# theogf/AugmentedGaussianProcesses.jl

Measured on AMD Instinct MI355X. Metric: cavi_iters_per_sec, higher is better.
Workload: dtype f64

## Files before the change

augmentedgaussianprocesses.jl_amd/csrc/agp_capi.hip:

```cpp
#include "../../include/agp_hip.h"

#include <hip/hip_runtime.h>

#include <algorithm>
#include <cmath>
#include <cstdio>
#include <cstring>
#include <string>
#include <vector>

#include "agp_cavi.h"
#include "agp_comm.h"
#include "agp_hyper.h"
#include "agp_kmeans.h"
#include "agp_linalg.h"

using namespace agp;

struct agp_ctx {
  int device = 0;
  hipStream_t stream = nullptr;
  std::string err;
  int32_t* dag_flags = nullptr;
  int64_t dag_cap = 0;
// ... 17 lines not shown
  int32_t* safe_retries = nullptr;
  int n_cu = 0;
  bool dag_off = false;
  int64_t dag_retries_seen = 0;
  int64_t dag_cooldown = 0, dag_backoff = 512;
  hipStream_t side = nullptr;
  hipEvent_t ev_fork = nullptr, ev_join = nullptr;
  void* chol_li = nullptr;
  size_t chol_li_bytes = 0;
  hipStream_t chain_stream = nullptr;
  int32_t* chain_go = nullptr;
  int32_t* chain_ctr = nullptr;
  int32_t chain_exits = 0;
  int chain_state = 0;
  int32_t chain_seq = 0;
};

#define HIPCHK(ctx, expr)                                                                       \
  do {                                                                                          \
    hipError_t _e = (expr);                                                                     \
    if (_e != hipSuccess) {                                                                     \
      (ctx)->err = std::string(#expr) + " : " + hipGetErrorString(_e);                          \
      return AGP_ERR_HIP;                                                                       \
    }                                                                                           \
  } while (0)

#define LAUNCHCHK(ctx)                                                                          \
  do {                                                                                          \
    hipError_t _e = hipGetLastError();                                                          \
    if (_e != hipSuccess) {                                                                     \
      (ctx)->err = std::string("kernel launch : ") + hipGetErrorString(_e) + " @" + std::to_string(__LINE__); \
// ... 158 lines not shown
  LAUNCHCHK(c);
  return AGP_OK;
}
template <typename T>
__global__ __launch_bounds__(CHOL_THREADS) void k_safe_rowstats(CholBatch<T> bt, SafeSrc<T> src, int64_t ld, int64_t ldx, int64_t lde,
                                                                int64_t ne, int64_t nt, int32_t* __restrict__ info, int64_t nvalid,
                                                                unsigned* __restrict__ bar, int32_t* __restrict__ retries,
                                                                int64_t B, int nslices, RowstatsBatch<T> rb, int64_t ldp,
                                                                int64_t ldw, int64_t cols, T jitter, T rho, LikParams<T> lp,
                                                                const T* __restrict__ y, const int64_t* __restrict__ idx,
                                                                T* __restrict__ Kt, T* __restrict__ muf, T* __restrict__ varf,
                                                                T* __restrict__ cb, T* __restrict__ theta, T* __restrict__ r,
                                                                T* __restrict__ w, int* __restrict__ flags,
                                                                const T* __restrict__ lam, T* __restrict__ gamma,
                                                                int rows_done = 0, const int32_t* __restrict__ pf_word = nullptr,
                                                                int32_t pf_want = 0) {
  __shared__ __attribute__((aligned(16))) T sm[3 * TILE * LDP];
  __shared__ __attribute__((aligned(16))) T sc[SC_ELEMS];
  __shared__ T piv[TILE];
  const bool ran = chol_safe_body<T>(bt, src, 1, ld, ldx, lde, ne, nt, info, nvalid, bar, retries, sm, sc, piv);
  if (ran || !rows_done) {
    const int64_t wpb = CHOL_THREADS / 64, nwave = (int64_t)gridDim.x * wpb;
    for (int64_t i = (int64_t)blockIdx.x * wpb + (threadIdx.x >> 6); i < B; i += nwave)
      rowstats_row<T>(i, threadIdx.x & 63, 0, B, nslices, rb, ldp, ldw, cols, jitter, rho, lp, y, idx, Kt, muf, varf, cb, theta, r,
                      w, (int64_t)0, flags, lam, gamma);
  }
  if (pf_word && blockIdx.x == 0 && threadIdx.x == 0) {
    long spins = 0;
    while ((int32_t)(__hip_atomic_load(pf_word, __ATOMIC_RELAXED, __HIP_MEMORY_SCOPE_SYSTEM) - pf_want) < 0) {
      __builtin_amdgcn_s_sleep(8);
      if (++spins > (1L << 27)) {
        atomicExch(info, -2);
        break;
      }
    }
  }
}

template <typename T>
__global__ __launch_bounds__(CHOL_THREADS) void k_safe_symv_trmv(CholBatch<T> bt, SafeSrc<T> src, int64_t ld, int64_t ldx, int64_t lde,
// ... 195 lines not shown
struct ProHost {
  const T* kap = nullptr;
  int64_t ldk = 0, Kdim = 0;
  const T *w = nullptr, *r = nullptr;
  T* eta2 = nullptr;
  const T* Kinv = nullptr;
  int64_t ldm = 0;
  T* eta1 = nullptr;
  const T* kinv_mu0 = nullptr;
  T lr = T(0);
  const T *packed = nullptr, *tred = nullptr;
  const int32_t* arrive = nullptr;
  int32_t arrive_want = 0;
  unsigned char grp[32] = {};
  T* Cout = nullptr;
};
static void pro_ks_table(int64_t nt, int64_t nq, bool f64, unsigned char* ks, unsigned char* kf) {
  const double tc = f64 ? 2.7 : 1.6, tau = f64 ? 17.8 : 14.0;
  for (int64_t c = 0; c < nt && c < 32; ++c) {
    int want;
    if (c == 0) want = 8;
    else if (c == 1) want = f64 ? 4 : 8;
    else want = (int)std::ceil((double)nq * (tc + 0.3) / (tau * (double)c - 12.0));
    want = std::max(1, std::min<int>(want, (int)std::min<int64_t>(8, nq)));
    ks[c] = kf[c] = (unsigned char)want;
  }
}
static bool dag_test_abort() {
  static const bool on = []() {
    const char* e = getenv("AGP_DAG_TEST_ABORT");
    return e && e[0] == '1';
  }();
  return on;
}

template <typename T>
static agp_status potrf_fused(agp_ctx* c, T* A, int64_t ld, int64_t n, T* X, int64_t ldx, T* Dg, T* E, int64_t lde,
                              int64_t ne, int do_x, int32_t* info_dev, int64_t nvalid, const T* erow = nullptr,
// ... 6 lines not shown
  const int64_t nt = n / TILE;
  const bool use_dag = chol_use_dag(c, nt, ne);
  bool split_used = false;
  if (pro && !(use_dag && X && !want_l && nt <= 32)) {
    c->err = "potrf_fused: a pending natural-gradient step can only ride on the CAVI step's task-graph launch";
    return AGP_ERR_INVALID;
  }
  if (use_dag && X) {
    const int64_t nx = (do_x && nt > 1) ? nt : 0;
    ProArgs<T> pa{};
    int64_t nhelp = 0;
    if (pro) {
      if (pro->packed)
        for (int64_t cc = 0; cc < nt; ++cc) pa.ks[cc] = pa.kf[cc] = 1;
      else
        pro_ks_table(nt, pro->Kdim / TILE, sizeof(T) == 8, pa.ks, pa.kf);
      for (int64_t cc = 0; cc < nt; ++cc) nhelp += pro_nhelp(nt, cc, pa.ks[cc], pa.kf[cc]);
    }
    const int64_t nf = ((nt + ne + nx) * nt + 3 * nt + 1 + nhelp) * DAG_FS;
    if (c->dag_cap < nf) {
      if (c->dag_flags) (void)hipFree(c->dag_flags);
      c->dag_flags = nullptr;
      c->dag_cap = 0;
      if (hipMalloc((void**)&c->dag_flags, sizeof(int32_t) * (size_t)(nf + 1024)) != hipSuccess) return AGP_ERR_NOMEM;
      c->dag_cap = nf + 1024;
      HIPCHK(c, hipMemsetAsync(c->dag_flags, 0, sizeof(int32_t) * (size_t)c->dag_cap, c->stream));
      c->dag_epoch = 0;
    }
    c->dag_epoch += 1;
    const int64_t ntiles = nt * (nt + 1) / 2 + ne * nt + (nx ? nt * (nt + 1) / 2 : 0);
    const int64_t hstride = ((2 * nt + ne) * nt + 3 * nt + nhelp) * TILE * TILE;
// ... 43 lines not shown
    one.E[0] = E;
    if (pro) {
      pa.kap = pro->kap;
      pa.ldk = pro->ldk;
      pa.Kdim = pro->Kdim;
      pa.w = pro->w;
      pa.r = pro->r;
      pa.eta2 = pro->eta2;
      pa.Kinv = pro->Kinv;
      pa.ldm = pro->ldm;
      pa.eta1 = pro->eta1;
      pa.kinv_mu0 = pro->kinv_mu0;
      pa.lr = pro->lr;
      pa.packed = pro->packed;
      pa.Cout = pro->Cout;
      pa.tred = pro->tred;
      pa.arrive = pro->arrive;
      pa.arrive_want = pro->arrive_want;
      memcpy(pa.grp, pro->grp, sizeof(pa.grp));
      pa.HS = H + (3 * nt + (nt + ne + nx) * nt) * TILE * TILE;
      pa.sflags = c->dag_flags + ((nt + ne + nx) * nt + 3 * nt + 1) * DAG_FS;
      const int other = hs ^ 1;
      if (c->hset[other] && c->h_dirty[other].on && c->h_dirty[other].nb == 1 && c->htype == (int)sizeof(T)) {
        pa.fill = (T*)c->hset[other];
        pa.fill_n = c->h_dirty[other].used;
        pa.nfill = 64;
        c->h_dirty[other].on = false;
      }
      unsigned long long* const ptrace = nullptr;
      constexpr unsigned lds_pad = 0;
      if (step_inst && chain_split_wanted(ntiles + nhelp, true, sizeof(T) == 8) && chain_split_ready(c)) {
        if (pa.Cout) {
          c->err = "potrf_fused: C = S + K^-1/4 (ProArgs::Cout) cannot ride on a split (chain kernel + tile kernel) launch";
          return AGP_ERR_INVALID;
        }
        chain_split_arm(c, ds, 1);
        split_used = true;
        hipLaunchKernelGGL((k_chol_dag<T, true, false, false, true, true, 1>), dim3(1), dim3(CHOL_THREADS), 0, c->chain_stream, one, 1,
                           (int64_t)0, ld, ldx, lde, ne, nt, info_dev, nvalid, c->dag_flags, c->dag_epoch, ptrace, H, hstride, nx, erow, 0,
                           ds, pa, epi ? *epi : EpiArgs<T>{});
        chain_split_wait_here(c);
        hipLaunchKernelGGL((k_chol_dag<T, true, false, false, true, true, 2>), dim3((unsigned)(ntiles + nhelp + pa.nfill)),
                           dim3(CHOL_THREADS), lds_pad, c->stream, one, 1, (int64_t)0, ld, ldx, lde, ne, nt, info_dev, nvalid,
                           c->dag_flags, c->dag_epoch, ptrace, H, hstride, nx, erow, 0, ds, pa, epi ? *epi : EpiArgs<T>{});
// ... 653 lines not shown
  int64_t ov_off[8] = {}, ov_cnt[8] = {};
  unsigned char ov_grp[32] = {};
  T *rbuf2 = nullptr, *wbuf2 = nullptr;
  struct SafeDeferred {
    bool on = false;
    CholBatch<T> bt{};
    SafeSrc<T> src{};
    RowstatsBatch<T> rb{};
    int64_t ne = 0, nt = 0, B = 0;
    int ns = 0;
    T rho = T(0);
    const T* y = nullptr;
    const int64_t* idx = nullptr;
    T *r = nullptr, *w = nullptr;
    unsigned grid = 1;
  } sdef;
  agp_status run_deferred_safe(const int32_t* pf_word = nullptr, int32_t pf_want = 0) {
    if (!sdef.on) return AGP_OK;
    sdef.on = false;
    hipLaunchKernelGGL((k_safe_rowstats<T>), dim3(sdef.grid), dim3(CHOL_THREADS), 0, st(), sdef.bt, sdef.src, mp, mp, mp, sdef.ne,
                       sdef.nt, info_dev, m, ctx->safe_bar, ctx->safe_retries, sdef.B, sdef.ns, sdef.rb, ldp, mp, mp, (T)jitter,
                       sdef.rho, lp, sdef.y, sdef.idx, Kt, muf, varf, cbuf, theta, sdef.r, sdef.w, flags_dev, (const T*)lam_dev,
                       gamma, 1, pf_word, pf_want);
    LAUNCHCHK(ctx);
    return AGP_OK;
  }
  bool epi_allowed() const {
    static const bool off = []() {
      const char* e = getenv("AGP_STEP_EPILOGUE");
      return e && e[0] == '0';
    }();
    if (off) return false;
    const int k = lp.kind;
    return (k == AGP_LIK_GAUSSIAN && !lp.noise_dev) || k == AGP_LIK_LOGISTIC || k == AGP_LIK_STUDENTT || k == AGP_LIK_LAPLACE ||
           k == AGP_LIK_BAYESIANSVM || k == AGP_LIK_NEGBINOMIAL;
  }
  bool pro_allowed() const {
    static const bool off = []() {
      const char* e = getenv("AGP_STEP_PROLOGUE");
      return e && e[0] == '0';
    }();
    if (off || nl != 1 || mo || mo_sharded) return false;
    if (mp / TILE > 16) return false;
    const int k = lp.kind;
    return k == AGP_LIK_GAUSSIAN || k == AGP_LIK_LOGISTIC || k == AGP_LIK_STUDENTT || k == AGP_LIK_LAPLACE ||
           k == AGP_LIK_BAYESIANSVM || k == AGP_LIK_NEGBINOMIAL || k == AGP_LIK_POISSON;
  }
  agp_status flush() override {
    AGPCHK(run_deferred_safe());
    if (!pend.on && !pendp.on) return AGP_OK;
    Latent& g = lat[0];
    g.C_valid = false;
    if (pend.on) {
      pend.on = false;
      AGPCHK((syrk_tn<T, SY_ETA2>(ctx, pend.kap, mp, mp, pend.Bq, pend.w, 0, g.La, mp, g.eta2, pend.Kinv, mp, pend.lr, pend.r,
                                  g.eta1, pend.kinv_mu0)));
    } else {
      pendp.on = false;
      if (pendp.overlap) {
        pendp.overlap = false;
        HIPCHK(ctx, hipStreamWaitEvent(st(), pendp.cm->ev_out, 0));
      }
      const int64_t ntri = (mp / TILE) * (mp / TILE + 1) / 2;
      hipLaunchKernelGGL((k_eta2_from_packed<T>), dim3((unsigned)(4 * ntri + (mp + 255) / 256)), dim3(256), 0, st(), stats + mp, mp,
                         g.eta2, pendp.Kinv, g.La, pendp.lr, ntri, (const T*)stats, pendp.kinv_mu0, g.eta1, mp);
    }
    LAUNCHCHK(ctx);
    g.la_state = 0;
    g.xa_valid = false;
    return AGP_OK;
  }
  agp_status step_finish() override {
    if (pro_allowed() && chol_use_dag(ctx, mp / TILE, rup64(B_last) / TILE + 1, 1) && mp / TILE <= 32) {
      Latent& g = lat[0];
      g.C_valid = false;
      pend.on = true;
      pend.Bq = rup64(B_last);
      pend.lr = (T)cur_lr();
      pend.kap = g.kappa;
      pend.Kinv = kinv_step(g);
      pend.kinv_mu0 = kinv_mu0_step(g);
      pend.r = rbuf;
      pend.w = wbuf;
      g.la_state = 1;
      g.xa_valid = false;
      g.post_valid = false;
      g.pred_valid = g.predvar_valid = false;
      n_opt += 1;
      return kappa_released();
    }
    AGPCHK(run_deferred_safe());
// ... 155 lines not shown
    }
    if (pf_fork) dcheck(hipEventDestroy(pf_fork), __LINE__);
    if (elbo_pin) {
      dcheck(hipHostFree(elbo_pin), __LINE__);
      for (auto& e : elbo_ev)
        if (e) dcheck(hipEventDestroy(e), __LINE__);
    }
    if (pf_stream) dcheck(hipStreamDestroy(pf_stream), __LINE__);
    for (auto q : sig)
      if (q) dcheck(hipFree(q), __LINE__);
    if (arrive_dev) dcheck(hipFree(arrive_dev), __LINE__);
    if (pf_done) dcheck(hipEventDestroy(pf_done), __LINE__);
    for (auto e : step_done)
      if (e) dcheck(hipEventDestroy(e), __LINE__);
    T* ps[] = {rbuf2, wbuf2, pw0, pw1, Kt, muf, varf, cbuf, theta, gamma, rbuf, wbuf, alpha, beta, gsum, alpha_save, emuf,
               evarf, stats, Tw, Tw2, tmpv, lr_dev, Kstar, ppm, ppv, pmu, pvar};
    for (T* p : ps)
      if (p) dfree(p);
    T* hps[] = {hyH1, hyH2, hyH3, hy_gmu, hy_gs, hy_muf, hy_pZ, hy_dZ, hyKap, hyKnm, hy_upart, hy_pZ2};
    for (T* p : hps)
      if (p) dfree(p);
    double* hds[] = {hy_pvar, hy_pscale, hy_g, hy_tied, hy_pvar2, hy_pscale2};
    for (double* p : hds)
      if (p) dfree(p);
    for (auto& g : lat) {
      free_online(g);
      T* sp[] = {g.sKinv, g.sXk, g.skinv_mu0, g.Cmat};
      for (T* q : sp)
        if (q) dfree(q);
      if (g.kadam) dfree(g.kadam);
      if (g.z_am) dfree(g.z_am);
// ... 423 lines not shown
    dag_tick(ctx);
    refresh_lazy = !fresh;
    const agp_status rks = refresh_K();
    refresh_lazy = false;
    AGPCHK(rks);
    const int64_t Bq = rup64(B);
    const int ns = (int)(2 * mp / TILE);
    const bool reuse = !desc.stochastic && !fresh && x == x_last && idx == idx_last && B == B_last && ldx == ldx_last;
    const bool reuse_eval = fresh && eval_cache_ok && x == ev_x && idx == ev_idx && B == ev_B && ldx == ev_ldx;
    if (!fresh)
      for (auto& g : lat) g.kappa_eval = false;
    const bool prefetched = pf_valid && !fresh && x == pf_x && idx == pf_idx && B == pf_B && ldx == pf_ldx;
    int dag_nb = 0;
    for (int q = DAG_MAX_NB; q >= 1 && !dag_nb; --q)
      if (chol_use_dag(ctx, mp / TILE, Bq / TILE + 1, q)) dag_nb = q;
    StepSync ssync{};
    const bool sync_step = sig_state == 1 && !fresh && nl == 1 && dag_nb > 0 &&
                           !(lat[0].la_state == 1 && lat[0].xa_valid);
    if (sync_step) {
      ssync.ds.started = sig[0];
      ssync.ds.seq = started_seq + 1;
    } else if (rel_pending) {
      AGPCHK(run_deferred_safe());
      slot_kind[rel_slot] = 0;
      HIPCHK(ctx, hipEventRecord(step_done[rel_slot], st()));
      rel_pending = false;
    }
    bool use_pro = false;
    if (pend.on || pendp.on) {
      use_pro = !fresh && nl == 1 && dag_nb > 0 && (prefetched || (reuse && lat[0].kappa_valid)) && pro_allowed() &&
                mp / TILE <= 32 && (pendp.on || pend.Bq >= TILE);
      if (!use_pro) AGPCHK(flush());
    }
    const bool use_epi = use_pro && in_cavi_step && epi_allowed();
    if (prefetched) {
      if (sig_state == 1) {
        if (sdef.on) {
          AGPCHK(run_deferred_safe((const int32_t*)sig[1], pf_seq));
        } else {
          hipLaunchKernelGGL(k_wait_ge_fast, dim3(1), dim3(64), 0, st(), (const int32_t*)sig[1], pf_seq, info_dev);
          LAUNCHCHK(ctx);
        }
      } else {
        AGPCHK(run_deferred_safe());
        HIPCHK(ctx, hipStreamWaitEvent(st(), pf_done, 0));
      }
      for (auto& g : lat) {
        std::swap(g.Knm, g.Knm_alt);
        std::swap(g.Wbuf, g.Wbuf_alt);
        std::swap(g.pk, g.pk_alt);
        T* left = g.kappa;
        g.kappa = g.kappa_alt;
        g.kappa_alt = g.kappa_old;
        g.kappa_old = left;
      }
      pf_valid = false;
    }
    AGPCHK(run_deferred_safe());
    CholBatch<T> merged_bt{};
    SafeSrc<T> merged_src{};
    bool merged_safe = false;
    for (int l = 0; l < nl; ++l) {
      Latent& g = lat[l];
      const bool keep = (reuse && g.kappa_valid) || (reuse_eval && g.kappa_eval);
      g.keep_last = keep;
      if (prefetched) {
      } else if (!keep) {
        AGPCHK(ensure_zsc(g));
        dim3 gk((unsigned)(mp / TILE), (unsigned)(Bq / TILE));
        (void)launch_kernelmatrix<T>(ctx, st(), (const T*)x, ldx, idx, B, (const T*)g.Z,
                           D, m, D, (const T*)g.scales, g.k.kind, kvar(g), g.Knm, mp, Bq, mp, 0, T(0),
                           (const T*)nullptr, (T*)nullptr, (int64_t)0, 0, (const T*)g.Zsc, (const T*)g.zn);
        LAUNCHCHK(ctx);
// ... 73 lines not shown
              ph.packed = stats + mp;
              ph.tred = stats;
              if (pendp.overlap) {
                ph.arrive = arrive_dev;
                ph.arrive_want = pendp.epoch;
                memcpy(ph.grp, ov_grp, sizeof(ph.grp));
              }
              ph.Kdim = 0;
              ph.Kinv = pendp.Kinv;
              ph.kinv_mu0 = pendp.kinv_mu0;
              ph.lr = pendp.lr;
            } else {
              ph.kap = pend.kap;
              ph.Kdim = pend.Bq;
              ph.w = pend.w;
              ph.r = pend.r;
              ph.Kinv = pend.Kinv;
              ph.kinv_mu0 = pend.kinv_mu0;
              ph.lr = pend.lr;
            }
          }
          EpiArgs<T> ea{};
          if (use_epi) {
            Latent& g0 = lat[0];
            std::swap(rbuf, rbuf2);
            std::swap(wbuf, wbuf2);
            ea.on = 1;
            ea.B = B;
            ea.nslices = ns;
            ea.pk = g0.pk;
// ... 8 lines not shown
            ea.idx = idx;
            ea.Kt = Kt;
            ea.muf = muf;
            ea.varf = varf;
            ea.cb = cbuf;
            ea.theta = theta;
            ea.r = rbuf;
            ea.w = wbuf;
            ea.flags = flags_dev;
            ea.lam = lam_dev;
            ea.gamma = gamma;
          }
          AGPCHK(potrf_fused<T>(ctx, bt.A[0], mp, mp, bt.X[0], mp, bt.Dg[0], bt.E[0], mp, nel, 0, info_dev, m,
                                (const T*)lat[todo[l0]].eta1, false, &src, &defer, sync_step ? &ssync : nullptr,
                                use_pro ? &ph : nullptr, use_epi ? &ea : nullptr));
          if (use_pro) {
            pend.on = pendp.on = pendp.overlap = false;
            n_prologue += 1;
          }
          merged_safe = defer;
          launches += dag_nb > 0 ? 1 : chol_launch_count(ntl, nel);
        } else if (dag_nb > 0) {
          AGPCHK(potrf_dag_batch<T>(ctx, bt, nb, mp, mp, mp, mp, nel, info_dev, m, &src));
          launches += 1;
        } else {
          AGPCHK(potrf_fused_batch<T>(ctx, bt, nb, mp, mp, mp, mp, nel, info_dev, m));
          launches += chol_launch_count(ntl, nel);
        }
      }
      if (!todo.empty()) AGPCHK(timing_end(launches));
// ... 25 lines not shown
        if (use_epi) {
          sdef.on = true;
          sdef.bt = merged_bt;
          sdef.src = merged_src;
          sdef.rb = rb;
          sdef.ne = ne_;
          sdef.nt = nt_;
          sdef.B = B;
          sdef.ns = ns;
          sdef.rho = (T)rho;
          sdef.y = (const T*)y;
          sdef.idx = idx;
          sdef.r = rbuf;
          sdef.w = wbuf;
          sdef.grid = g1;
          continue;
        }
        hipLaunchKernelGGL((k_safe_rowstats<T>), dim3(g1), dim3(CHOL_THREADS), 0, st(), merged_bt, merged_src, mp, mp, mp, ne_, nt_,
                           info_dev, m, ctx->safe_bar, ctx->safe_retries, B, ns, rb, ldp, mp, mp, (T)jitter, (T)rho, lp, (const T*)y,
                           idx, Kt, muf, varf, cbuf, theta, rbuf, wbuf, flags_dev, (const T*)lam_dev, gamma);
        LAUNCHCHK(ctx);
        continue;
      }
      const dim3 grid((unsigned)((B * 64 + 255) / 256), (unsigned)nb);
      hipLaunchKernelGGL((k_rowstats_local<T>), grid, dim3(256), 0, st(), B, ns, rb, ldp, mp, mp, (T)jitter, (T)rho, lp,
                         (const T*)y, idx, Kt + l0 * Bp, muf + l0 * Bp, varf + l0 * Bp, cbuf + l0 * Bp, theta + l0 * Bp,
                         rbuf + l0 * Bp, wbuf + l0 * Bp, Bp, flags_dev, (const T*)lam_dev, gamma + l0 * Bp);
      LAUNCHCHK(ctx);
    }
    AGPCHK(lik_tail(y, idx, B, rho, fresh));
// ... 1020 lines not shown
    if (tail) {
      tail->on = defer;
      if (defer) {
        tail->bt = CholBatch<T>{};
        tail->bt.A[0] = g.La;
        tail->bt.X[0] = g.Xa;
        tail->bt.Dg[0] = g.DgA;
        tail->bt.E[0] = g.Wbuf;
        tail->src = src;
        tail->ne = Bq / TILE + 1;
        tail->nt = mp / TILE;
      }
    }
    if (use_pro) {
      pend.on = false;
      n_prologue += 1;
      if (ph.Cout) {
        g.C_valid = true;
        g.C_kap = ph.kap;
      }
    }
    AGPCHK(timing_end(chol_use_dag(ctx, mp / TILE, Bq / TILE + 1) ? 1 : chol_launch_count(mp / TILE, Bq / TILE + 1)));
    g.la_state = 1;
    g.xa_valid = with_x != 0;
    if (with_x) g.xa_epoch += 1;
    g.sigma_epoch = sigma_done ? g.xa_epoch : -1;
    return AGP_OK;
  }

  agp_status refactor(Latent& g) {
// ... 25 lines not shown
    if (fused) AGPCHK(kappa_released());
    return AGP_OK;
  }
  agp_status kappa_released() {
    if (pf_stream) {
      if (rel_pending) {
        slot_kind[rel_slot] = 0;
        HIPCHK(ctx, hipEventRecord(step_done[rel_slot], st()));
        rel_pending = false;
      }
      step_parity ^= 1;
      if (sig_state == 1 && nl == 1) {
        rel_pending = true;
        rel_slot = step_parity ^ 1;
      } else {
        AGPCHK(run_deferred_safe());
        slot_kind[step_parity ^ 1] = 0;
        HIPCHK(ctx, hipEventRecord(step_done[step_parity ^ 1], st()));
      }
    }
    return AGP_OK;
  }

  agp_status check_status() override {
    int32_t words[4] = {0, 0, 0, 0};
    HIPCHK(ctx, hipMemcpyAsync(words, info_dev, sizeof(words), hipMemcpyDeviceToHost, st()));
    HIPCHK(ctx, hipStreamSynchronize(st()));
    const int32_t info = words[0], infoK = words[1], orderK = words[3];
    const int flags = (int)words[2];
    dag_retry_check(ctx);
    if (info != 0 || flags != 0) {
// ... 807 lines not shown
    }
    if (overlap) {
      if (cm->ctx != ctx) {
        ctx->err = "agp_comm belongs to another ctx (its collectives would run on another stream)";
        return AGP_ERR_INVALID;
      }
      AGPCHK(overlap_groups());
      arrive_epoch += 1;
      AGPCHK(comm_allreduce_groups(cm, stats, (int)sizeof(T), ov_off, ov_cnt, ov_ng, sizeof(T) == 8 ? AGP_F64 : AGP_F32, arrive_dev,
                                   arrive_epoch));
    } else
      AGPCHK(comm_sum(cm, stats, (int64_t)nl * stats_stride()));
    if (merge) {
      Latent& g = lat[0];
      pendp.on = true;
      pendp.overlap = overlap;
      pendp.epoch = arrive_epoch;
      pendp.cm = cm;
      pendp.lr = (T)cur_lr();
      pendp.Kinv = kinv_step(g);
      pendp.kinv_mu0 = kinv_mu0_step(g);
      g.la_state = 1;
      g.xa_valid = false;
      g.post_valid = false;
      g.pred_valid = g.predvar_valid = false;
      n_opt += 1;
      return AGP_OK;
    }
    return step_global(false);
  }
// ... 505 lines not shown
  {
    DevGuard guard(device);
    int cur = -1;
    if (hipGetDevice(&cur) != hipSuccess || cur != device) return AGP_ERR_HIP;
  }
  agp_ctx* c = new agp_ctx();
  c->device = device;
  c->stream = (hipStream_t)hip_stream;
  *out = c;
  return AGP_OK;
}

agp_status agp_ctx_destroy(agp_ctx* ctx) {
  if (!ctx) return AGP_OK;
  DevGuard guard(ctx->device);
  if (ctx->tri_scratch || ctx->dag_flags || ctx->hset[0]) {
    (void)hipStreamSynchronize(ctx->stream);
    if (ctx->dag_flags) (void)hipFree(ctx->dag_flags);
    for (int q = 0; q < 2; ++q)
      if (ctx->hset[q]) (void)hipFree(ctx->hset[q]);
    if (ctx->tri_scratch) (void)hipFree(ctx->tri_scratch);
  }
  if (ctx->kmm_scratch) (void)hipFree(ctx->kmm_scratch);
  if (ctx->bal_ws) {
    (void)hipStreamSynchronize(ctx->stream);
    (void)hipFree(ctx->bal_ws);
  }
  if (ctx->chain_stream) {
    (void)hipStreamSynchronize(ctx->chain_stream);
    (void)hipStreamDestroy(ctx->chain_stream);
// ... 1140 lines not shown
```

augmentedgaussianprocesses.jl_amd/csrc/agp_chol.h:

```cpp
#pragma once
#include "agp_cavi.h"
#include "agp_device.h"

namespace agp {

constexpr int LDP = TILE + 2;
#ifndef AGP_PIVOT_ALG
#define AGP_PIVOT_ALG 0
#endif
constexpr int CHOL_THREADS = 512;

__device__ __forceinline__ double rcp1(double p) {
  double r = __builtin_amdgcn_rcp(p);
  return fma(r, fma(-p, r, 1.0), r);
}
__device__ __forceinline__ double rsqrt1(double p) {
  double y = __builtin_amdgcn_rsq(p);
  const double h = 0.5 * p;
  y = y * fma(-h * y, y, 1.5);
  y = y * fma(-h * y, y, 1.5);
  return y;
}
__device__ __forceinline__ float rsqrt1(float p) {
  float y = __builtin_amdgcn_rsqf(p);
// ... 1352 lines not shown
  const T* kinv_mu0 = nullptr;
  T lr = T(0);
  T* HS = nullptr;
  int32_t* sflags = nullptr;
  T* fill = nullptr;
  int64_t fill_n = 0;
  int32_t nfill = 0;
  const T* packed = nullptr;
  const T* tred = nullptr;
  const int32_t* arrive = nullptr;
  int32_t arrive_want = 0;
  unsigned char grp[32] = {};
  unsigned char ks[32] = {};
  unsigned char kf[32] = {};
  T* Cout = nullptr;
};

constexpr int ARRIVE_STRIDE = 16;
__device__ __forceinline__ void pro_arrival_gate(const int32_t* arrive, int g, int32_t want, int32_t* info) {
  if (threadIdx.x == 0) {
    long spins = 0;
    while ((int32_t)(__hip_atomic_load(arrive + g * ARRIVE_STRIDE, __ATOMIC_RELAXED, __HIP_MEMORY_SCOPE_AGENT) - want) < 0) {
      __builtin_amdgcn_s_sleep(8);
      if (++spins > (1L << 23)) {
        atomicExch(info, -4);
        break;
      }
    }
  }
  __syncthreads();
  __builtin_amdgcn_fence(__ATOMIC_ACQUIRE, "agent");
// ... 49 lines not shown
#endif
template <typename T, int ROLE, bool PRO>
constexpr int dag_min_waves() {
  return ROLE != 2 ? 1 : PRO ? (sizeof(T) == 8 ? 2 : 4) : (sizeof(T) == 8 ? AGP_TILES_WAVES_F64 : AGP_TILES_WAVES_F32);
}
template <typename T>
struct ProdArgs {
  T* out = nullptr;
  int64_t ld = 0;
  int64_t base = 0;
  T* fill = nullptr;
  int64_t fill_n = 0;
  double* ld_out = nullptr;
  int32_t* status = nullptr;
};

template <typename T, bool FUSED, bool BATCH = false, bool TRACE = false, bool STEP = false, bool PRO = false, int ROLE = 0>
__global__ __launch_bounds__(CHOL_THREADS, (dag_min_waves<T, ROLE, PRO>()))
void k_chol_dag(CholBatch<T> bt, int nb, int64_t fstride, int64_t ld, int64_t ldx,
                                                           int64_t lde, int64_t ne, int64_t nt,
                                                           int32_t* __restrict__ info, int64_t nvalid, int32_t* flags,
                                                           int32_t epoch, unsigned long long* trace, T* H, int64_t hstride,
                                                           int64_t nx_, const T* __restrict__ erow, int opts, DagSync sync,
                                                           ProArgs<T> pro = ProArgs<T>{}, EpiArgs<T> epi = EpiArgs<T>{},
                                                           ProdArgs<T> prod = ProdArgs<T>{}) {
  static_assert(!PRO || (FUSED && !BATCH), "the prologue exists for single-problem launches with a chain workgroup only");
  static_assert(ROLE == 0 || (FUSED && STEP && !TRACE), "the split launch exists for the CAVI step's launches");
  const int64_t nx = STEP ? 0 : nx_;
  const int write_x = STEP ? 0 : (opts & 1);
  const bool store_l = STEP ? false : (opts & 2) != 0;
// ... 35 lines not shown
#endif
          break;
        }
      }
    }
    __syncthreads();
    if (!wait_ok) {
      chain_count_out(sync);
      return;
    }
    __builtin_amdgcn_fence(__ATOMIC_ACQUIRE, "agent");
  }
  T* bufA = sm;
  T* bufB = sm + TILE * LDP;
  const int tid = threadIdx.x;
  int64_t b = bidx, c = 0;
  bool helper = false;
  int64_t hbase = 0;
  const bool is_prod = !BATCH && !STEP && ROLE != 1 && prod.out != nullptr && bidx >= prod.base;
  static_assert(ROLE == 0 || STEP, "product workgroups (ProdArgs) must reach their sentinel refill unconditionally: ROLE 0 only");
  if (is_prod) {
    b = 0;
  } else if (PRO && ROLE == 1) {
  } else if (PRO) {
    for (;;) {
      if (c == nt) {
        const T sv = __builtin_bit_cast(T, Sent<T>::bits);
        for (int64_t i = b * CHOL_THREADS + tid; i < pro.fill_n; i += (int64_t)pro.nfill * CHOL_THREADS) pro.fill[i] = sv;
        return;
      }
      const int64_t nh = pro_nhelp(nt, c, pro.ks[c], pro.kf[c]), ntile = nt - c + ne + (nx ? c + 1 : 0);
      if (b < nh) {
        helper = true;
        break;
      }
      b -= nh;
      if (b < ntile) break;
      b -= ntile;
      hbase += nh;
      ++c;
    }
  } else {
    while (b >= nt - c + ne + (nx ? c + 1 : 0)) {
      b -= nt - c + ne + (nx ? c + 1 : 0);
      ++c;
    }
  }
#define PRO_TS(i) \
  if (PRO && trace && tid == 0) trace[i] = wall_clock64()
  if (PRO && helper) {
    const int64_t ntc = nt - c, nn = ntc < PRO_NEAR ? ntc : PRO_NEAR;
    const int kfc = pro.kf[c], kso = pro.ks[c];
    const bool near = b < nn * (kfc - 1);
    const int ksc = near ? kfc : kso;
    const int64_t bo = near ? b : b - nn * (kfc - 1);
    const int64_t tb = (near ? 0 : nn) + bo / (ksc - 1), sl = 1 + bo % (ksc - 1), nq = pro.Kdim / TILE;
    Acc8<T> S;
    S.zero();
    if (c == 0 && b == 0) PRO_TS(1024);
    pro_slice<T>(pro.kap, pro.ldk, pro.w, (c + tb) * TILE, c * TILE, sl * nq / ksc, (sl + 1) * nq / ksc, sm, S);
    if (c == 0 && b == 0) PRO_TS(1025);
    T* hs = pro.HS + (hbase + b) * (TILE * TILE);
    {
      int e = 0;
      acc8_foreach<T>(S, [&](int r, int cc, T& val) {
        (void)r;
        (void)cc;
        __hip_atomic_store(hs + pro_slot_off<T>(tid, e++), val, __ATOMIC_RELAXED, __HIP_MEMORY_SCOPE_AGENT);
      });
    }
    dag_signal(pro.sflags + (hbase + b) * DAG_FS, epoch);
// ... 69 lines not shown
    return;
  }
  DAG_TR(0);
  const bool chain = FUSED && c == 0 && b == 0;
  if (STEP && !BATCH && sync.started && chain && tid == 0 && ROLE != 1)
    __hip_atomic_store(sync.started, sync.seq, __ATOMIC_RELAXED, __HIP_MEMORY_SCOPE_SYSTEM);
  if (ROLE == 2 && chain) {
    if (tid == 0 && sync.go) __hip_atomic_store(sync.go, sync.go_val, __ATOMIC_RELAXED, __HIP_MEMORY_SCOPE_SYSTEM);
    if (!PRO) return;
  }
  if (ROLE == 1 && !chain) return;
  Acc8<T> acc;
  if (PRO && ROLE == 1) {
  } else if (PRO && !ext) {
    const int64_t ntc_ = nt - c, nn_ = ntc_ < PRO_NEAR ? ntc_ : PRO_NEAR;
    const int ksc = b < nn_ ? pro.kf[c] : pro.ks[c];
    const int64_t nq = pro.Kdim / TILE;
    const int tsb = chain ? 0 : (R < 4 && c < 4) ? 64 + 8 * (4 * (int)R + (int)c) : 2040;
    PRO_TS(tsb);
    acc.zero();
    pro_slice<T>(pro.kap, pro.ldk, pro.w, R * TILE, c0, 0, nq / ksc, sm, acc);
    if (pro.packed) {
      if (pro.arrive) pro_arrival_gate(pro.arrive, pro.grp[c], pro.arrive_want, info);
      const T* __restrict__ tp = pro.packed + pack_index(R, c, nt) * (TILE * TILE);
      acc8_foreach<T>(acc, [&](int r, int cc, T& val) { val = tp[r * TILE + cc]; });
    }
    PRO_TS(tsb + 1);
    Acc8<T> e2v, kiv;
    acc8_foreach<T>(e2v, [&](int r, int cc, T& val) { val = pro.eta2[(R * TILE + r) * pro.ldm + c0 + cc]; });
    acc8_foreach<T>(kiv, [&](int r, int cc, T& val) { val = pro.Kinv[(R * TILE + r) * pro.ldm + c0 + cc]; });
    if (ksc > 1) {
      const int64_t h0 = hbase + (b < nn_ ? b * (pro.kf[c] - 1) : nn_ * (pro.kf[c] - 1) + (b - nn_) * (pro.ks[c] - 1));
      if (tid < ksc - 1) {
        long spins = 0;
        while (__hip_atomic_load(pro.sflags + (h0 + tid) * DAG_FS, __ATOMIC_RELAXED, __HIP_MEMORY_SCOPE_AGENT) != epoch) {
          __builtin_amdgcn_s_sleep(1);
// ... 159 lines not shown
        }
#pragma unroll
        for (int q = 0; q < TILE * TILE / CHOL_THREADS; ++q) {
          const int e = tl + q * CHOL_THREADS;
          __hip_atomic_store(HX + k * SLOT + e, xv[q], __ATOMIC_RELAXED, __HIP_MEMORY_SCOPE_AGENT);
          if (write_x) X[(k0 + (e >> 6)) * ldx + k0 + (e & 63)] = xv[q];
        }
      }
      if (k + 1 == nt) {
        for (int e = tid; e < TILE * TILE; e += CHOL_THREADS) {
          if (ROLE == 1) __hip_atomic_store(Dg + k * TILE * TILE + e, bufA[(e >> 6) * LDP + (e & 63)], __ATOMIC_RELAXED, __HIP_MEMORY_SCOPE_AGENT);
          else Dg[k * TILE * TILE + e] = bufA[(e >> 6) * LDP + (e & 63)];
        }
        dag_signal(xready + k * DAG_FS, epoch);
        DAG_TRC(k, 3);
        if (ROLE == 1) chain_count_out(sync);
        return;
      }
      const bool late_feed = !pf_ok || pf_bad;
      if (late_feed) {
        dag_signal(xready + k * DAG_FS, epoch);
        DAG_TRC(k, 3);
        if (!dag_wait(pf.f1, pf.f2, epoch, abortf, info, &wait_ok)) {
          if (ROLE == 1) chain_count_out(sync);
          return;
        }
        load_tiles_lds_hv2<T>(HP + 2 * (k + 1) * SLOT, bufC, HP + (2 * (k + 1) + 1) * SLOT, bufD);
        __syncthreads();
      }
      if (TRACE && tid == 0) trace[chain_slot(k + 1, nt, ne, nx) * 8 + 7] = (unsigned long long)pf_ok;
// ... 112 lines not shown
    __syncthreads();
    factor_diag_tile_2lvl<T>(bufA, bufB, sc, piv, info, c0, nvalid);
    DAG_TR(2);
    for (int e = tid; e < TILE * TILE; e += CHOL_THREADS) {
      const int r = e >> 6, cc = e & 63;
      __hip_atomic_store(HX + c * SLOT + e, bufB[r * LDP + cc], __ATOMIC_RELAXED, __HIP_MEMORY_SCOPE_AGENT);
      X[(c0 + r) * ldx + c0 + cc] = bufB[r * LDP + cc];
    }
    dag_signal(xready + c * DAG_FS, epoch);
    for (int e = tid; e < TILE * TILE; e += CHOL_THREADS) Dg[c * TILE * TILE + e] = bufA[(e >> 6) * LDP + (e & 63)];
    DAG_TR(3);
    return;
  }
  if (!dag_wait(xready + c * DAG_FS, nullptr, epoch, abortf, info, &wait_ok)) return;
  DAG_TR(2);
  load_tile_lds_hv<T>(HX + c * SLOT, bufB);
  __syncthreads();
  DAG_TR(6);
  Acc8<T> out;
  out.zero();
  mma8<T>(bufA, bufB, out);
  {
    T* hs = HL + (R * nt + c) * SLOT;
    acc8_foreach<T>(out, [&](int r, int cc, T& val) {
      __hip_atomic_store(hs + r * TILE + cc, val, __ATOMIC_RELAXED, __HIP_MEMORY_SCOPE_AGENT);
    });
  }
  if (idr) {
    const int64_t i0 = (R - nt - ne) * TILE;
    acc8_foreach<T>(out, [&](int r, int cc, T& val) { X[(c0 + cc) * ldx + i0 + r] = val; });
  } else if (ext || store_l) {
    acc8_foreach<T>(out, [&](int r, int cc, T& val) { rowp[r * ldr + c0 + cc] = val; });
  }
  DAG_TR(7);
  dag_signal(ready + (R * nt + c) * DAG_FS, epoch);
  DAG_TR(3);
  if (epi_row) {
    __syncthreads();
    acc8_foreach<T>(out, [&](int r, int cc, T& val) { bufA[r * LDP + cc] = val; });
    __syncthreads();
    epi_acc(bufA, HL + ((nt + ne - 1) * nt + c) * SLOT);
    const int64_t i = (R - nt) * TILE + er;
    T sk = epi_sk;
#pragma unroll
    for (int o = 1; o < 8; o <<= 1) {
      epi_ss += __shfl_xor(epi_ss, o);
      epi_dt += __shfl_xor(epi_dt, o);
      sk += __shfl_xor(sk, o);
    }
    if ((tid & 7) == 0 && i < epi.B) {
      const T kd = epi.kdiag < T(0) ? epi.kd_ptr[0] : epi.kdiag;
      rowstats_finish<T>(i, epi_ss, epi_dt, sk, kd, epi.use_kt, epi.jitter, epi.rho, epi.lp, epi.y, epi.idx, epi.Kt, epi.muf,
                         epi.varf, epi.cb, epi.theta, epi.r, epi.w, epi.flags, epi.lam, epi.gamma, &epi_y);
    }
  }
#undef DAG_TR
#undef DAG_TRC
#undef PRO_TS
}

template <typename T>
__global__ void k_fill_sent(T* __restrict__ p, int64_t n, int64_t stride) {
  const T sv = __builtin_bit_cast(T, Sent<T>::bits);
  T* q = p + blockIdx.y * stride;
  for (int64_t i = blockIdx.x * (int64_t)blockDim.x + threadIdx.x; i < n; i += (int64_t)gridDim.x * blockDim.x) q[i] = sv;
}

template <typename T>
__global__ __launch_bounds__(NTHREADS) void k_trtri_level(const T* __restrict__ A, int64_t ld, T* __restrict__ X, int64_t ldx,
// ... 60 lines not shown
```

Measured before the change: 3178.

## Precompute leading prologue tiles in deferred safe-rowstats kernel for f64

When the deferred safe Cholesky/rowstats kernel runs and its Cholesky body did no work, it now precomputes the weighted kappa^T W kappa products for the first 2x2 prologue tiles into a scratch buffer, split into four K-slices, using MFMA. The following fused DAG prologue then sums these precomputed slices for those tiles instead of recomputing them, skips their helper blocks, and raises the helper split table head parameter to match. This moves work off the critical start of the next step's Cholesky chain into an earlier kernel, at the cost of extra work and a validity flag in that kernel plus more bookkeeping for when the buffer is current. Optional step-trace instrumentation is also added behind a compile-time flag.

```diff
diff --git a/augmentedgaussianprocesses.jl_amd/csrc/agp_capi.hip b/augmentedgaussianprocesses.jl_amd/csrc/agp_capi.hip
--- a/augmentedgaussianprocesses.jl_amd/csrc/agp_capi.hip
+++ b/augmentedgaussianprocesses.jl_amd/csrc/agp_capi.hip
@@ -55,7 +55,44 @@
   int32_t chain_exits = 0;
   int chain_state = 0;
   int32_t chain_seq = 0;
+  unsigned long long* strace = nullptr;
+  unsigned long long* strace_last = nullptr;
+  int64_t strace_n = 0;
 };
+
+#ifdef AGP_STEP_TRACE
+constexpr int64_t STRACE_RECS = 1024;
+static unsigned long long* step_trace_next(agp_ctx* c) {
+  static const char* path = getenv("AGP_STEP_TRACE");
+  if (!path || !path[0]) return nullptr;
+  const size_t bytes = sizeof(unsigned long long) * STRACE_SLOTS * STRACE_RECS;
+  if (!c->strace) {
+    if (hipMalloc((void**)&c->strace, bytes) != hipSuccess) return c->strace = nullptr;
+    (void)hipMemsetAsync(c->strace, 0, bytes, c->stream);
+  }
+  return c->strace + (c->strace_n++ % STRACE_RECS) * STRACE_SLOTS;
+}
+static void step_trace_dump(agp_ctx* c) {
+  const char* path = getenv("AGP_STEP_TRACE");
+  if (!c->strace || !path) return;
+  const int64_t n = std::min<int64_t>(c->strace_n, STRACE_RECS);
+  std::vector<unsigned long long> h((size_t)(STRACE_SLOTS * STRACE_RECS));
+  (void)hipDeviceSynchronize();
+  (void)hipMemcpy(h.data(), c->strace, h.size() * sizeof(unsigned long long), hipMemcpyDeviceToHost);
+  if (FILE* f = fopen(path, "wb")) {
+    const int64_t hdr[2] = {n, STRACE_SLOTS};
+    fwrite(hdr, sizeof(hdr), 1, f);
+    for (int64_t i = c->strace_n - n; i < c->strace_n; ++i)
+      fwrite(h.data() + (i % STRACE_RECS) * STRACE_SLOTS, sizeof(unsigned long long), STRACE_SLOTS, f);
+    fclose(f);
+  }
+  (void)hipFree(c->strace);
+  c->strace = nullptr;
+}
+#else
+static unsigned long long* step_trace_next(agp_ctx*) { return nullptr; }
+static void step_trace_dump(agp_ctx*) {}
+#endif
 
 #define HIPCHK(ctx, expr)                                                                       \
   do {                                                                                          \
@@ -244,16 +281,29 @@
                                                                 T* __restrict__ w, int* __restrict__ flags,
                                                                 const T* __restrict__ lam, T* __restrict__ gamma,
                                                                 int rows_done = 0, const int32_t* __restrict__ pf_word = nullptr,
-                                                                int32_t pf_want = 0) {
+                                                                int32_t pf_want = 0, const T* __restrict__ s00_kap = nullptr,
+                                                                int64_t s00_ldk = 0, int64_t s00_K = 0,
+                                                                const T* __restrict__ s00_w = nullptr, T* __restrict__ pre = nullptr,
+                                                                unsigned long long* trace = nullptr) {
   __shared__ __attribute__((aligned(16))) T sm[3 * TILE * LDP];
   __shared__ __attribute__((aligned(16))) T sc[SC_ELEMS];
   __shared__ T piv[TILE];
+#ifdef AGP_STEP_TRACE
+  if (trace && threadIdx.x == 0 && blockIdx.x < 256) trace[STRACE_SAFE0 + blockIdx.x] = wall_clock64();
+  StraceExit strace_exit{(trace && blockIdx.x < 256) ? trace + STRACE_SAFE1 + blockIdx.x : nullptr};
+#else
+  (void)trace;
+#endif
   const bool ran = chol_safe_body<T>(bt, src, 1, ld, ldx, lde, ne, nt, info, nvalid, bar, retries, sm, sc, piv);
   if (ran || !rows_done) {
     const int64_t wpb = CHOL_THREADS / 64, nwave = (int64_t)gridDim.x * wpb;
     for (int64_t i = (int64_t)blockIdx.x * wpb + (threadIdx.x >> 6); i < B; i += nwave)
       rowstats_row<T>(i, threadIdx.x & 63, 0, B, nslices, rb, ldp, ldw, cols, jitter, rho, lp, y, idx, Kt, muf, varf, cb, theta, r,
                       w, (int64_t)0, flags, lam, gamma);
+  }
+  if (pro_pre_on<T>() && pre) {
+    if (!ran) pro_pre_prepare<T>(s00_kap, s00_ldk, s00_K, s00_w, pre, sm);
+    if (blockIdx.x == 0 && threadIdx.x == 0) pre[PRO_PRE_VALID] = ran ? T(0) : T(1);
   }
   if (pf_word && blockIdx.x == 0 && threadIdx.x == 0) {
     long spins = 0;
@@ -479,14 +529,15 @@
   int32_t arrive_want = 0;
   unsigned char grp[32] = {};
   T* Cout = nullptr;
+  const T* pre = nullptr;
 };
-static void pro_ks_table(int64_t nt, int64_t nq, bool f64, unsigned char* ks, unsigned char* kf) {
-  const double tc = f64 ? 2.7 : 1.6, tau = f64 ? 17.8 : 14.0;
+static void pro_ks_table(int64_t nt, int64_t nq, bool f64, unsigned char* ks, unsigned char* kf, bool pre = false) {
+  const double tc = f64 ? 2.7 : 1.6, tau = f64 ? 17.8 : 14.0, head = pre ? 24.0 : 12.0;
   for (int64_t c = 0; c < nt && c < 32; ++c) {
     int want;
     if (c == 0) want = 8;
     else if (c == 1) want = f64 ? 4 : 8;
-    else want = (int)std::ceil((double)nq * (tc + 0.3) / (tau * (double)c - 12.0));
+    else want = (int)std::ceil((double)nq * (tc + 0.3) / std::max(tau * (double)c - head, 1.0));
     want = std::max(1, std::min<int>(want, (int)std::min<int64_t>(8, nq)));
     ks[c] = kf[c] = (unsigned char)want;
   }
@@ -523,7 +574,7 @@
       if (pro->packed)
         for (int64_t cc = 0; cc < nt; ++cc) pa.ks[cc] = pa.kf[cc] = 1;
       else
-        pro_ks_table(nt, pro->Kdim / TILE, sizeof(T) == 8, pa.ks, pa.kf);
+        pro_ks_table(nt, pro->Kdim / TILE, sizeof(T) == 8, pa.ks, pa.kf, pro->pre != nullptr);
       for (int64_t cc = 0; cc < nt; ++cc) nhelp += pro_nhelp(nt, cc, pa.ks[cc], pa.kf[cc]);
     }
     const int64_t nf = ((nt + ne + nx) * nt + 3 * nt + 1 + nhelp) * DAG_FS;
@@ -597,6 +648,7 @@
       pa.lr = pro->lr;
       pa.packed = pro->packed;
       pa.Cout = pro->Cout;
+      pa.pre = pro->pre;
       pa.tred = pro->tred;
       pa.arrive = pro->arrive;
       pa.arrive_want = pro->arrive_want;
@@ -610,7 +662,8 @@
         pa.nfill = 64;
         c->h_dirty[other].on = false;
       }
-      unsigned long long* const ptrace = nullptr;
+      unsigned long long* const ptrace = step_inst ? step_trace_next(c) : nullptr;
+      c->strace_last = ptrace;
       constexpr unsigned lds_pad = 0;
       if (step_inst && chain_split_wanted(ntiles + nhelp, true, sizeof(T) == 8) && chain_split_ready(c)) {
         if (pa.Cout) {
@@ -1294,15 +1347,32 @@
     const int64_t* idx = nullptr;
     T *r = nullptr, *w = nullptr;
     unsigned grid = 1;
+    unsigned long long* trace = nullptr;
   } sdef;
-  agp_status run_deferred_safe(const int32_t* pf_word = nullptr, int32_t pf_want = 0) {
+  T* s00buf = nullptr;
+  struct {
+    bool on = false;
+    const T *kap = nullptr, *w = nullptr;
+    int64_t K = 0;
+  } s00_for;
+  agp_status run_deferred_safe(const int32_t* pf_word = nullptr, int32_t pf_want = 0, bool want_s00 = false) {
     if (!sdef.on) return AGP_OK;
     sdef.on = false;
+    s00_for.on = false;
+    const bool s00 = pro_pre_on<T>() && want_s00 && pend.on && !pendp.on && pend.w == sdef.w && pend.Bq >= TILE && pend.Bq % TILE == 0;
+    if (s00 && !s00buf) AGPCHK(dmalloc<T>(ctx, &s00buf, PRO_PRE_VALID + 16));
     hipLaunchKernelGGL((k_safe_rowstats<T>), dim3(sdef.grid), dim3(CHOL_THREADS), 0, st(), sdef.bt, sdef.src, mp, mp, mp, sdef.ne,
                        sdef.nt, info_dev, m, ctx->safe_bar, ctx->safe_retries, sdef.B, sdef.ns, sdef.rb, ldp, mp, mp, (T)jitter,
                        sdef.rho, lp, sdef.y, sdef.idx, Kt, muf, varf, cbuf, theta, sdef.r, sdef.w, flags_dev, (const T*)lam_dev,
-                       gamma, 1, pf_word, pf_want);
+                       gamma, 1, pf_word, pf_want, s00 ? pend.kap : nullptr, (int64_t)mp, s00 ? pend.Bq : 0,
+                       s00 ? (const T*)pend.w : nullptr, s00 ? s00buf : nullptr, sdef.trace);
     LAUNCHCHK(ctx);
+    if (s00) {
+      s00_for.on = true;
+      s00_for.kap = pend.kap;
+      s00_for.w = pend.w;
+      s00_for.K = pend.Bq;
+    }
     return AGP_OK;
   }
   bool epi_allowed() const {
@@ -1328,6 +1398,7 @@
   }
   agp_status flush() override {
     AGPCHK(run_deferred_safe());
+    s00_for.on = false;
     if (!pend.on && !pendp.on) return AGP_OK;
     Latent& g = lat[0];
     g.C_valid = false;
@@ -1355,6 +1426,7 @@
       Latent& g = lat[0];
       g.C_valid = false;
       pend.on = true;
+      s00_for.on = false;
       pend.Bq = rup64(B_last);
       pend.lr = (T)cur_lr();
       pend.kap = g.kappa;
@@ -1540,7 +1612,7 @@
     for (auto e : step_done)
       if (e) dcheck(hipEventDestroy(e), __LINE__);
     T* ps[] = {rbuf2, wbuf2, pw0, pw1, Kt, muf, varf, cbuf, theta, gamma, rbuf, wbuf, alpha, beta, gsum, alpha_save, emuf,
-               evarf, stats, Tw, Tw2, tmpv, lr_dev, Kstar, ppm, ppv, pmu, pvar};
+               evarf, stats, Tw, Tw2, tmpv, lr_dev, Kstar, ppm, ppv, pmu, pvar, s00buf};
     for (T* p : ps)
       if (p) dfree(p);
     T* hps[] = {hyH1, hyH2, hyH3, hy_gmu, hy_gs, hy_muf, hy_pZ, hy_dZ, hyKap, hyKnm, hy_upart, hy_pZ2};
@@ -1994,6 +2066,10 @@
     int dag_nb = 0;
     for (int q = DAG_MAX_NB; q >= 1 && !dag_nb; --q)
       if (chol_use_dag(ctx, mp / TILE, Bq / TILE + 1, q)) dag_nb = q;
+    const bool take_pend = (pend.on || pendp.on) && !fresh && nl == 1 && dag_nb > 0 &&
+                           (prefetched || (reuse && lat[0].kappa_valid)) && pro_allowed() && mp / TILE <= 32 &&
+                           (pendp.on || pend.Bq >= TILE);
+    const bool pre_want = take_pend && in_cavi_step && epi_allowed();
     StepSync ssync{};
     const bool sync_step = sig_state == 1 && !fresh && nl == 1 && dag_nb > 0 &&
                            !(lat[0].la_state == 1 && lat[0].xa_valid);
@@ -2001,28 +2077,27 @@
       ssync.ds.started = sig[0];
       ssync.ds.seq = started_seq + 1;
     } else if (rel_pending) {
-      AGPCHK(run_deferred_safe());
+      AGPCHK(run_deferred_safe(nullptr, 0, pre_want));
       slot_kind[rel_slot] = 0;
       HIPCHK(ctx, hipEventRecord(step_done[rel_slot], st()));
       rel_pending = false;
     }
     bool use_pro = false;
     if (pend.on || pendp.on) {
-      use_pro = !fresh && nl == 1 && dag_nb > 0 && (prefetched || (reuse && lat[0].kappa_valid)) && pro_allowed() &&
-                mp / TILE <= 32 && (pendp.on || pend.Bq >= TILE);
+      use_pro = take_pend;
       if (!use_pro) AGPCHK(flush());
     }
-    const bool use_epi = use_pro && in_cavi_step && epi_allowed();
+    const bool use_epi = pre_want;
     if (prefetched) {
       if (sig_state == 1) {
         if (sdef.on) {
-          AGPCHK(run_deferred_safe((const int32_t*)sig[1], pf_seq));
+          AGPCHK(run_deferred_safe((const int32_t*)sig[1], pf_seq, use_epi));
         } else {
           hipLaunchKernelGGL(k_wait_ge_fast, dim3(1), dim3(64), 0, st(), (const int32_t*)sig[1], pf_seq, info_dev);
           LAUNCHCHK(ctx);
         }
       } else {
-        AGPCHK(run_deferred_safe());
+        AGPCHK(run_deferred_safe(nullptr, 0, use_epi));
         HIPCHK(ctx, hipStreamWaitEvent(st(), pf_done, 0));
       }
       for (auto& g : lat) {
@@ -2036,7 +2111,7 @@
       }
       pf_valid = false;
     }
-    AGPCHK(run_deferred_safe());
+    AGPCHK(run_deferred_safe(nullptr, 0, use_epi));
     CholBatch<T> merged_bt{};
     SafeSrc<T> merged_src{};
     bool merged_safe = false;
@@ -2140,6 +2215,8 @@
               ph.kap = pend.kap;
               ph.Kdim = pend.Bq;
               ph.w = pend.w;
+              if (use_epi && s00_for.on && s00_for.kap == pend.kap && s00_for.w == pend.w && s00_for.K == pend.Bq)
+                ph.pre = s00buf;
               ph.r = pend.r;
               ph.Kinv = pend.Kinv;
               ph.kinv_mu0 = pend.kinv_mu0;
@@ -2178,6 +2255,7 @@
           AGPCHK(potrf_fused<T>(ctx, bt.A[0], mp, mp, bt.X[0], mp, bt.Dg[0], bt.E[0], mp, nel, 0, info_dev, m,
                                 (const T*)lat[todo[l0]].eta1, false, &src, &defer, sync_step ? &ssync : nullptr,
                                 use_pro ? &ph : nullptr, use_epi ? &ea : nullptr));
+          s00_for.on = false;
           if (use_pro) {
             pend.on = pendp.on = pendp.overlap = false;
             n_prologue += 1;
@@ -2233,6 +2311,7 @@
           sdef.r = rbuf;
           sdef.w = wbuf;
           sdef.grid = g1;
+          sdef.trace = ctx->strace_last;
           continue;
         }
         hipLaunchKernelGGL((k_safe_rowstats<T>), dim3(g1), dim3(CHOL_THREADS), 0, st(), merged_bt, merged_src, mp, mp, mp, ne_, nt_,
@@ -3283,6 +3362,7 @@
     }
     if (use_pro) {
       pend.on = false;
+      s00_for.on = false;
       n_prologue += 1;
       if (ph.Cout) {
         g.C_valid = true;
@@ -3338,7 +3418,7 @@
         rel_pending = true;
         rel_slot = step_parity ^ 1;
       } else {
-        AGPCHK(run_deferred_safe());
+        AGPCHK(run_deferred_safe(nullptr, 0, true));
         slot_kind[step_parity ^ 1] = 0;
         HIPCHK(ctx, hipEventRecord(step_done[step_parity ^ 1], st()));
       }
@@ -4176,6 +4256,7 @@
     if (merge) {
       Latent& g = lat[0];
       pendp.on = true;
+      s00_for.on = false;
       pendp.overlap = overlap;
       pendp.epoch = arrive_epoch;
       pendp.cm = cm;
@@ -4711,6 +4792,7 @@
 agp_status agp_ctx_destroy(agp_ctx* ctx) {
   if (!ctx) return AGP_OK;
   DevGuard guard(ctx->device);
+  step_trace_dump(ctx);
   if (ctx->tri_scratch || ctx->dag_flags || ctx->hset[0]) {
     (void)hipStreamSynchronize(ctx->stream);
     if (ctx->dag_flags) (void)hipFree(ctx->dag_flags);
diff --git a/augmentedgaussianprocesses.jl_amd/csrc/agp_chol.h b/augmentedgaussianprocesses.jl_amd/csrc/agp_chol.h
--- a/augmentedgaussianprocesses.jl_amd/csrc/agp_chol.h
+++ b/augmentedgaussianprocesses.jl_amd/csrc/agp_chol.h
@@ -1390,7 +1390,56 @@
   unsigned char ks[32] = {};
   unsigned char kf[32] = {};
   T* Cout = nullptr;
+  const T* pre = nullptr;
 };
+
+constexpr int PRO_PRE_KS = 4, PRO_PRE_VALID = 3 * PRO_PRE_KS * TILE * TILE;
+template <typename T>
+constexpr bool pro_pre_on() { return sizeof(T) == 8; }
+__host__ __device__ __forceinline__ bool pro_pre_tile(int64_t R, int64_t c) { return R <= 1 && c <= 1; }
+template <typename T>
+__device__ __forceinline__ void pro_pre_prepare(const T* __restrict__ kap, int64_t ldk, int64_t K, const T* __restrict__ w,
+                                                T* __restrict__ out, T* red) {
+  typedef typename Mfma<T>::acc_t acc_t;
+  constexpr int NW = CHOL_THREADS / 64;
+  const int lane = threadIdx.x & 63, wave = threadIdx.x >> 6;
+  for (int u = blockIdx.x; u < 3 * PRO_PRE_KS * 16; u += gridDim.x) {
+    const int sl = u / (PRO_PRE_KS * 16), q = (u / 16) % PRO_PRE_KS, bi = (u >> 2) & 3, bj = u & 3;
+    const int64_t R0 = sl == 0 ? 0 : TILE, c0 = sl == 2 ? TILE : 0;
+    if (R0 + TILE > ldk) continue;
+    const int64_t kq0 = K * q / PRO_PRE_KS, kq1 = K * (q + 1) / PRO_PRE_KS;
+    const int64_t k0 = kq0 + (kq1 - kq0) * wave / NW, k1 = kq0 + (kq1 - kq0) * (wave + 1) / NW;
+    const T* __restrict__ pa = kap + R0 + 16 * bi + (lane & 15);
+    const T* __restrict__ pb = kap + c0 + 16 * bj + (lane & 15);
+    acc_t acc;
+#pragma unroll
+    for (int r = 0; r < 4; ++r) acc[r] = T(0);
+    constexpr int U = 8;
+    for (int64_t kb = k0; kb < k1; kb += 4 * U) {
+      T av[U], bv[U], wv[U];
+#pragma unroll
+      for (int j = 0; j < U; ++j) {
+        const int64_t kk = kb + 4 * j + (lane >> 4), kc = kk < k1 ? kk : k0;
+        wv[j] = kk < k1 ? w[kc] : T(0);
+        av[j] = pa[kc * ldk];
+        bv[j] = pb[kc * ldk];
+      }
+#pragma unroll
+      for (int j = 0; j < U; ++j) acc = Mfma<T>::mma(wv[j] * av[j], bv[j], acc);
+    }
+#pragma unroll
+    for (int r = 0; r < 4; ++r) red[wave * 256 + Mfma<T>::row(lane, r) * 16 + (lane & 15)] = acc[r];
+    __syncthreads();
+    if (threadIdx.x < 256) {
+      const int e = threadIdx.x;
+      T v = red[e];
+#pragma unroll
+      for (int o = 1; o < NW; ++o) v += red[o * 256 + e];
+      out[(int64_t)(sl * PRO_PRE_KS + q) * TILE * TILE + (16 * bi + (e >> 4)) * TILE + 16 * bj + (e & 15)] = v;
+    }
+    __syncthreads();
+  }
+}
 
 constexpr int ARRIVE_STRIDE = 16;
 __device__ __forceinline__ void pro_arrival_gate(const int32_t* arrive, int g, int32_t want, int32_t* info) {
@@ -1470,6 +1519,21 @@
   double* ld_out = nullptr;
   int32_t* status = nullptr;
 };
+
+constexpr int STRACE_SLOTS = 8192, STRACE_XPUB = 600, STRACE_EXT = 1100, STRACE_FILL0 = 1400, STRACE_FILL1 = 1500, STRACE_WG0 = 2048,
+              STRACE_WG1 = 4096, STRACE_MAXWG = 2048, STRACE_SAFE0 = 6144, STRACE_SAFE1 = 6400;
+#ifdef AGP_STEP_TRACE
+struct StraceExit {
+  unsigned long long* p;
+  __device__ ~StraceExit() {
+    if (p && threadIdx.x == 0) *p = wall_clock64();
+  }
+};
+#define STRACE(i) \
+  if (PRO && ROLE == 0 && trace && threadIdx.x == 0) trace[i] = wall_clock64()
+#else
+#define STRACE(i)
+#endif
 
 template <typename T, bool FUSED, bool BATCH = false, bool TRACE = false, bool STEP = false, bool PRO = false, int ROLE = 0>
 __global__ __launch_bounds__(CHOL_THREADS, (dag_min_waves<T, ROLE, PRO>()))
@@ -1535,6 +1599,10 @@
   T* bufA = sm;
   T* bufB = sm + TILE * LDP;
   const int tid = threadIdx.x;
+#ifdef AGP_STEP_TRACE
+  StraceExit strace_exit{(PRO && ROLE == 0 && trace && bidx < STRACE_MAXWG) ? trace + STRACE_WG1 + bidx : nullptr};
+  if (bidx < STRACE_MAXWG) STRACE(STRACE_WG0 + bidx);
+#endif
   int64_t b = bidx, c = 0;
   bool helper = false;
   int64_t hbase = 0;
@@ -1547,7 +1615,9 @@
     for (;;) {
       if (c == nt) {
         const T sv = __builtin_bit_cast(T, Sent<T>::bits);
+        if (b < 64) STRACE(STRACE_FILL0 + b);
         for (int64_t i = b * CHOL_THREADS + tid; i < pro.fill_n; i += (int64_t)pro.nfill * CHOL_THREADS) pro.fill[i] = sv;
+        if (b < 64) STRACE(STRACE_FILL1 + b);
         return;
       }
       const int64_t nh = pro_nhelp(nt, c, pro.ks[c], pro.kf[c]), ntile = nt - c + ne + (nx ? c + 1 : 0);
@@ -1576,6 +1646,7 @@
     const int ksc = near ? kfc : kso;
     const int64_t bo = near ? b : b - nn * (kfc - 1);
     const int64_t tb = (near ? 0 : nn) + bo / (ksc - 1), sl = 1 + bo % (ksc - 1), nq = pro.Kdim / TILE;
+    if (pro_pre_on<T>() && pro.pre && pro_pre_tile(c + tb, c)) return;
     Acc8<T> S;
     S.zero();
     if (c == 0 && b == 0) PRO_TS(1024);
@@ -1675,12 +1746,35 @@
   if (PRO && ROLE == 1) {
   } else if (PRO && !ext) {
     const int64_t ntc_ = nt - c, nn_ = ntc_ < PRO_NEAR ? ntc_ : PRO_NEAR;
-    const int ksc = b < nn_ ? pro.kf[c] : pro.ks[c];
+    const bool pre = pro_pre_on<T>() && pro.pre && pro_pre_tile(R, c);
+    const int ksc = pre ? 1 : b < nn_ ? pro.kf[c] : pro.ks[c];
     const int64_t nq = pro.Kdim / TILE;
     const int tsb = chain ? 0 : (R < 4 && c < 4) ? 64 + 8 * (4 * (int)R + (int)c) : 2040;
     PRO_TS(tsb);
     acc.zero();
-    pro_slice<T>(pro.kap, pro.ldk, pro.w, R * TILE, c0, 0, nq / ksc, sm, acc);
+    if (pre && pro.pre[PRO_PRE_VALID] == T(1)) {
+      const T* __restrict__ pp = pro.pre + (R + c) * PRO_PRE_KS * TILE * TILE;
+      T pv[PRO_PRE_KS][8];
+      int e = 0;
+      acc8_foreach<T>(acc, [&](int r, int cc, T& val) {
+        (void)val;
+#pragma unroll
+        for (int q = 0; q < PRO_PRE_KS; ++q) pv[q][e] = pp[q * TILE * TILE + r * TILE + cc];
+        ++e;
+      });
+      e = 0;
+      acc8_foreach<T>(acc, [&](int r, int cc, T& val) {
+        (void)r;
+        (void)cc;
+        T v = pv[0][e];
+#pragma unroll
+        for (int q = 1; q < PRO_PRE_KS; ++q) v += pv[q][e];
+        val = v;
+        ++e;
+      });
+    } else {
+      pro_slice<T>(pro.kap, pro.ldk, pro.w, R * TILE, c0, 0, nq / ksc, sm, acc);
+    }
     if (pro.packed) {
       if (pro.arrive) pro_arrival_gate(pro.arrive, pro.grp[c], pro.arrive_want, info);
       const T* __restrict__ tp = pro.packed + pack_index(R, c, nt) * (TILE * TILE);
@@ -1870,6 +1964,7 @@
         }
         dag_signal(xready + k * DAG_FS, epoch);
         DAG_TRC(k, 3);
+        STRACE(STRACE_XPUB);
         if (ROLE == 1) chain_count_out(sync);
         return;
       }
@@ -2012,6 +2107,9 @@
   }
   if (!dag_wait(xready + c * DAG_FS, nullptr, epoch, abortf, info, &wait_ok)) return;
   DAG_TR(2);
+  const bool strace_row = ext && !idr && c == nt - 1 && R - nt < 64;
+  (void)strace_row;
+  if (strace_row) STRACE(STRACE_EXT + 4 * (R - nt));
   load_tile_lds_hv<T>(HX + c * SLOT, bufB);
   __syncthreads();
   DAG_TR(6);
@@ -2033,11 +2131,13 @@
   DAG_TR(7);
   dag_signal(ready + (R * nt + c) * DAG_FS, epoch);
   DAG_TR(3);
+  if (strace_row) STRACE(STRACE_EXT + 4 * (R - nt) + 1);
   if (epi_row) {
     __syncthreads();
     acc8_foreach<T>(out, [&](int r, int cc, T& val) { bufA[r * LDP + cc] = val; });
     __syncthreads();
     epi_acc(bufA, HL + ((nt + ne - 1) * nt + c) * SLOT);
+    STRACE(STRACE_EXT + 4 * (R - nt) + 2);
     const int64_t i = (R - nt) * TILE + er;
     T sk = epi_sk;
 #pragma unroll
@@ -2051,6 +2151,10 @@
       rowstats_finish<T>(i, epi_ss, epi_dt, sk, kd, epi.use_kt, epi.jitter, epi.rho, epi.lp, epi.y, epi.idx, epi.Kt, epi.muf,
                          epi.varf, epi.cb, epi.theta, epi.r, epi.w, epi.flags, epi.lam, epi.gamma, &epi_y);
     }
+#ifdef AGP_STEP_TRACE
+    __syncthreads();
+    STRACE(STRACE_EXT + 4 * (R - nt) + 3);
+#endif
   }
 #undef DAG_TR
 #undef DAG_TRC
```

After: 3241 (median of 6 runs). +2.0%, better.
